# HopperLogger/HopperRender

Measured on AMD Instinct MI355X. Metric: interpolated frames/sec + ms/flow-calc, 2160p HDR, 1/2/4/8 MI355X, higher is better.
Workload: dtype u16

## Files before the change

### hopperrender_amd/csrc/hf_flow.hip

```cpp
#include <utility>
#include "hf_kernels.h"
#include "hf_phase_plane.h"

namespace hf {

thread_local LaunchObserver* t_launch_observer = nullptr;

namespace {

__device__ __forceinline__ int clampi(int v, int lo, int hi) { return min(max(v, lo), hi); }

__device__ __forceinline__ int rel_offset(int layer, int R) {
    const int d = layer - (R >> 1);
    return d > 0 ? d * d : -(d * d);
}

__device__ __forceinline__ int mirror_clamp(int p, int dim) {
    if (p >= dim) p = 2 * dim - p - 1; else if (p < 0) p = -p - 1;
    return clampi(p, 0, dim - 1);
}

template <typename E>
__global__ __launch_bounds__(256) void prep_phase_kernel(const PrepBatch batch, int H, int W, int S, PhaseLayout pl) {
    const E* __restrict__ f = (const E*)batch.frame[blockIdx.y];
// ... 802 lines not shown
        if (a.prev2.tx) {
            gx = table_at(a.prev2.tx, a.prev2, wx << a.cur.log2w, wy << a.cur.log2w);
            gy = table_at(a.prev2.ty, a.prev2, wx << a.cur.log2w, wy << a.cur.log2w);
        }
#pragma unroll
        for (int ax = 0; ax < 2; ax++)
#pragma unroll
            for (int v = 0; v < NV; v++) pre[ax][v] = tab0[ax * tab_axis + v];
        zx = wc.ox == gx; zy = wc.oy == gy;
    }
    if (a.pend.active) {
        const int tx0 = tile.tx * M::TW, ty0 = tile.ty * M::TH;
        const bool leader = tid == 0 && (tx0 & (a.pend.lvl.window - 1)) == 0 && (ty0 & (a.pend.lvl.window - 1)) == 0;
        const int v = resolve_pending(g, a, tx0, ty0, lane, leader);
        if (a.pend.axis) wc.oy = v; else wc.ox = v;
    }
    const int cap_cz = 7;
    uint32_t captured = 0;
    int off[2] = {wc.ox, wc.oy};

#pragma unroll
    for (int axis = 0; axis < 2; axis++) {
        bool reuse = zy && (axis == 0 ? zx : off[0] == wc.ox);
        if constexpr (G == 64) reuse = __builtin_amdgcn_readfirstlane((int)reuse) != 0;
        if (a.counters) {
            const bool lead = WS == 32 ? tid == 0 : G == 2 ? (lane & M::XM) == 0 : (lane & (G - 1)) == 0;
            const uint64_t mw = __builtin_amdgcn_ballot_w64(lead), mr = __builtin_amdgcn_ballot_w64(lead && reuse);
            if (lane == 0 && mw) {
                uint32_t* const c = a.counters + kCounterLevels + 4 * (a.level_index & 15) + 2 * axis;
                atomicAdd(c, (uint32_t)__builtin_popcountll(mw));
                if (mr) atomicAdd(c + 1, (uint32_t)__builtin_popcountll(mr));
            }
        }
        flow_v4* const tab = tab0 + axis * tab_axis;
        uint32_t tot[NOWN];
        int first = 0;
        if constexpr (PX == 4 && NR == 1) {
            uint32_t W[8];
            if (!reuse) {
                Strip<PX> strip[NR];
#pragma unroll
                for (int r = 0; r < NR; r++) strip[r] = load_strip<PX, true>(g, a, cx0, cy + r);
                uint32_t p[16];
#pragma unroll
                for (int cz = 0; cz < 16; cz++) p[cz] = 0u;
                bool from_lds = false;
                if constexpr (WS == 16 && SPLIT) {
                    if (axis == 1) from_lds = ysads_tile_try<16, 4, 1, true, kTabGroups>(p, g, a, strip[0].ref, off[0], off[1], cx0, cy, lane, s_rows);
                } else if constexpr (WS == 8 && SPLIT) {
                    if (axis == 1) from_lds = ysads_win8_try<true, kTabGroups>(p, g, a, strip[0].ref, off[0], off[1], cx0, cy, lane, s_rows);
                } else if constexpr (WS == 32) {
                    if (axis == 1) from_lds = ysads_tile_try<32, 8, 4, true, kTabGroups>(p, g, a, strip[0].ref, off[0], off[1], cx0 - lx, cy - ly, tid, s_rows);
                }
                if (!from_lds) strip_sads<4, G == 64, true, true, true, kTabGroups>(p, g, a, strip[0], off[0], off[1], axis);
                const uint32_t selw = (cy & 1) ? 0x07060302u : 0x05040100u;
#pragma unroll
                for (int j = 0; j < 8; j++) {
                    const uint32_t q0 = p[2 * j] + lane_xor<M::RM>(p[2 * j], lane);
                    const uint32_t q1 = p[2 * j + 1] + lane_xor<M::RM>(p[2 * j + 1], lane);
                    W[j] = __builtin_amdgcn_perm(q1, q0, selw);
                }
                if (a.sad_write) { tab[0] = flow_v4{W[0], W[1], W[2], W[3]}; tab[1] = flow_v4{W[4], W[5], W[6], W[7]}; }
            } else {
                const flow_v4 lo = pre[axis][0], hi = pre[axis][1];
                W[0] = lo.x; W[1] = lo.y; W[2] = lo.z; W[3] = lo.w; W[4] = hi.x; W[5] = hi.y; W[6] = hi.z; W[7] = hi.w;
            }
            first = packed_reduce<G, M::XM>(W, tot, lane);
        } else if constexpr (PX == 4) {
            uint32_t V[8];
            if (!reuse) {
                Strip<PX> strip[NR];
#pragma unroll
                for (int r = 0; r < NR; r++) strip[r] = load_strip<PX, true>(g, a, cx0, cy + r);
                uint32_t p[16];
#pragma unroll
                for (int cz = 0; cz < 16; cz++) p[cz] = 0u;
#pragma unroll
                for (int r = 0; r < NR; r++) strip_sads<4, false, true, true, true, kTabGroups>(p, g, a, strip[r], off[0], off[1], axis);
                uint32_t W0[8], W1[8];
#pragma unroll
                for (int j = 0; j < 8; j++) {
                    W0[j] = __builtin_amdgcn_perm(p[2 * j + 1], p[2 * j], 0x05040100u);
                    W1[j] = __builtin_amdgcn_perm(p[2 * j + 1], p[2 * j], 0x07060302u);
                    V[j] = W0[j] + W1[j];
                }
                if (a.sad_write) {
                    tab[0] = flow_v4{W0[0], W0[1], W0[2], W0[3]}; tab[1] = flow_v4{W0[4], W0[5], W0[6], W0[7]};
                    tab[2] = flow_v4{W1[0], W1[1], W1[2], W1[3]}; tab[3] = flow_v4{W1[4], W1[5], W1[6], W1[7]};
                }
            } else {
                const flow_v4 a0 = pre[axis][0], a1 = pre[axis][1], b0 = pre[axis][2 % NV], b1 = pre[axis][3 % NV];
                V[0] = a0.x + b0.x; V[1] = a0.y + b0.y; V[2] = a0.z + b0.z; V[3] = a0.w + b0.w;
                V[4] = a1.x + b1.x; V[5] = a1.y + b1.y; V[6] = a1.z + b1.z; V[7] = a1.w + b1.w;
            }
            first = packed_reduce<G, M::XM>(V, tot, lane);
        } else if constexpr (NR == 2) {
            if (!reuse) {
                Strip<PX> strip[NR];
#pragma unroll
                for (int r = 0; r < NR; r++) strip[r] = load_strip<PX, true>(g, a, cx0, cy + r);
#pragma unroll
                for (int cz = 0; cz < 16; cz++) tot[cz] = 0u;
#pragma unroll
                for (int r = 0; r < NR; r++) strip_sads<PX, false, true, false, true, kTabGroups>(tot, g, a, strip[r], off[0], off[1], axis);
            } else {
                unpack_u16x8(pre[axis][0], tot); unpack_u16x8(pre[axis][1 % NV], tot + 8);
            }
        } else {
            if (!reuse) {
                Strip<PX> strip[NR];
#pragma unroll
                for (int r = 0; r < NR; r++) strip[r] = load_strip<PX, true>(g, a, cx0, cy + r);
                uint32_t sad[16];
#pragma unroll
                for (int cz = 0; cz < 16; cz++) sad[cz] = 0u;
                strip_sads<PX, false, true, false, true, kTabGroups>(sad, g, a, strip[0], off[0], off[1], axis);
                butterfly_level<16, M::XM>(sad, lane);
#pragma unroll
                for (int k = 0; k < 8; k++) tot[k] = sad[k];
            } else {
                unpack_u16x8(pre[axis][0], tot);
            }
            first = (lane & M::XM) ? 8 : 0;
        }
        if constexpr (WS == 32) {
            if ((lane & 3) == 0) s_part[axis][wave][first] = tot[0];
            __syncthreads();
            tot[0] = s_part[axis][0][first] + s_part[axis][1][first] + s_part[axis][2][first] + s_part[axis][3][first];
        }
        const int best = group_argmin<G, true, M::XM>(tot, first, a, off[axis], axis ? wc.nby : wc.nbx, wc.npix, cap_cz,
                                                      axis == 0 && a.capture_delta, captured, lane);
        off[axis] = (int)(int16_t)(off[axis] + rel_offset(best, 16));
    }

    const bool leader = WS == 32 ? tid == 0 : G == 2 ? (lane & M::XM) == 0 : (lane & (G - 1)) == 0;
    HF_DBG_CHECK(wx >= 0 && wy >= 0 && wx < a.cur.nwx && wy < a.cur.nwy, 105);
    if (leader) {
        a.cur.tx[wy * a.cur.nwx + wx] = (int16_t)off[0];
        a.cur.ty[wy * a.cur.nwx + wx] = (int16_t)off[1];
        if (WS == 32 && a.still_count && off[0] == wc.ox && off[1] == wc.oy) atomicAdd(a.still_count, 1u);
        if (a.capture_delta && wx == 0 && wy == 0) *a.total_delta = captured / a.delta_divisor;
    }
}

template <bool FULL, bool R16, int NH>
__device__ __forceinline__ void flow_level32_wave_body(const Geom& g, const FlowStep& a, const TileId& tile, [[maybe_unused]] uint32_t* s_rows) {
    using M = Map<32>;
    const int R = R16 ? 16 : a.R;
    const int lane = (int)threadIdx.x;
    int lx, ly;
    M::at(lane, lx, ly);
    const int tx0 = tile.tx * M::TW, ty0 = tile.ty * M::TH;
    const int cx0 = tx0 + lx;
    const int wx = tx0 >> a.cur.log2w, wy = ty0 >> a.cur.log2w;
    WinConst wc = load_win_const(g, a, wx, wy, false);
    if (a.pend.active) {
        const bool leader = lane == 0 && (tx0 & (a.pend.lvl.window - 1)) == 0 && (ty0 & (a.pend.lvl.window - 1)) == 0;
        const int v = resolve_pending(g, a, tx0, ty0, lane, leader);
        if (a.pend.axis) wc.oy = v; else wc.ox = v;
    }
    const int cap_cz = (R >> 1) - 1;
    uint32_t captured = 0;
    int off[2] = {wc.ox, wc.oy};
#pragma unroll
    for (int axis = 0; axis < 2; axis++) {
        uint32_t sad[16];
#pragma unroll
        for (int cz = 0; cz < 16; cz++) sad[cz] = 0u;
        bool staged = false;
        if constexpr (FULL) if (axis == 1) {
            staged = ytile_can_stage<32>(g, a, __builtin_amdgcn_readfirstlane(off[1]), ty0);
            if (staged) with_rs(g.rs, [&](auto RS) { ystage_copy<decltype(RS)::value, 32, 8, 1>(a, __builtin_amdgcn_readfirstlane(off[0]), __builtin_amdgcn_readfirstlane(off[1]), tx0, ty0, lane, s_rows); });
        }
#pragma unroll 1
        for (int v = 0; v < 4; v++) {
            const Strip<4> strip = load_strip<4, FULL>(g, a, cx0, ty0 + ly + 8 * v);
            if (staged) with_rs(g.rs, [&](auto RS) { ystage_sads<decltype(RS)::value, 32, 8, 1, false, NH>(sad, a, strip.ref, __builtin_amdgcn_readfirstlane(off[0]), v * 64 + lane, s_rows); });
            else strip_sads<4, true, FULL, false, R16, NH>(sad, g, a, strip, off[0], off[1], axis);
        }
        const int first = group_reduce<64, 1>(sad, lane);
        const int best = group_argmin<64, R16, 1>(sad, first, a, off[axis], axis ? wc.nby : wc.nbx, wc.npix, cap_cz,
                                                  axis == 0 && a.capture_delta, captured, lane);
        off[axis] = (int)(int16_t)(off[axis] + rel_offset(best, R));
    }
    HF_DBG_CHECK(wx >= 0 && wy >= 0 && wx < a.cur.nwx && wy < a.cur.nwy, 105);
    if (lane == 0) {
        a.cur.tx[wy * a.cur.nwx + wx] = (int16_t)off[0];
        a.cur.ty[wy * a.cur.nwx + wx] = (int16_t)off[1];
        if (a.capture_delta && wx == 0 && wy == 0) *a.total_delta = captured / a.delta_divisor;
        if (a.still_count && off[0] == wc.ox && off[1] == wc.oy) atomicAdd(a.still_count, 1u);
    }
}

__device__ __forceinline__ void flow_level32_wave_tab_body(const Geom& g, const FlowStep& a, const TileId& tile, [[maybe_unused]] uint32_t* s_rows) {
    using M = Map<32>;
    const int lane = (int)threadIdx.x;
    int lx, ly;
    M::at(lane, lx, ly);
    const int tx0 = tile.tx * M::TW, ty0 = tile.ty * M::TH;
    const int cx0 = tx0 + lx, cy_0 = ty0 + ly;
    const int wx = tx0 >> a.cur.log2w, wy = ty0 >> a.cur.log2w;
    WinConst wc = load_win_const(g, a, wx, wy, false);
    const int nblk = a.sad_nbx * a.sad_nby;
    const int blk = (cy_0 >> 1) * a.sad_nbx + (cx0 >> 1) + (cy_0 & 1);
    HF_DBG_CHECK(blk >= 0 && blk + 12 * a.sad_nbx < nblk, 110);
    flow_v4* const tab0 = (flow_v4*)a.sadtab + (size_t)blk * 2;
    const size_t tab_axis = (size_t)nblk * 2, tab_round = (size_t)a.sad_nbx * 8;
    if (a.pend.active) {
        const bool leader = lane == 0 && (tx0 & (a.pend.lvl.window - 1)) == 0 && (ty0 & (a.pend.lvl.window - 1)) == 0;
        const int v = resolve_pending(g, a, tx0, ty0, lane, leader);
        if (a.pend.axis) wc.oy = v; else wc.ox = v;
    }
    const int cap_cz = 7;
    uint32_t captured = 0;
    int off[2] = {wc.ox, wc.oy};
    const uint32_t selw = (cy_0 & 1) ? 0x07060302u : 0x05040100u;
#pragma unroll
    for (int axis = 0; axis < 2; axis++) {
        if (a.counters && lane == 0) atomicAdd(a.counters + kCounterLevels + 4 * (a.level_index & 15) + 2 * axis, 1u);
        flow_v4* const tab = tab0 + axis * tab_axis;
        bool staged = false;
        if (axis == 1) {
            staged = ytile_can_stage<32>(g, a, __builtin_amdgcn_readfirstlane(off[1]), ty0);
            if (staged) with_rs(g.rs, [&](auto RS) { ystage_copy<decltype(RS)::value, 32, 8, 1>(a, __builtin_amdgcn_readfirstlane(off[0]), __builtin_amdgcn_readfirstlane(off[1]), tx0, ty0, lane, s_rows); });
        }
        uint32_t total = 0;
        int first = 0;
#pragma unroll 1
        for (int v = 0; v < 4; v++) {
            const Strip<4> strip = load_strip<4, true>(g, a, cx0, cy_0 + 8 * v);
            uint32_t p[16];
#pragma unroll
            for (int cz = 0; cz < 16; cz++) p[cz] = 0u;
            if (staged) with_rs(g.rs, [&](auto RS) { ystage_sads<decltype(RS)::value, 32, 8, 1, true, kTabGroups>(p, a, strip.ref, __builtin_amdgcn_readfirstlane(off[0]), v * 64 + lane, s_rows); });
            else strip_sads<4, true, true, true, true, kTabGroups>(p, g, a, strip, off[0], off[1], axis);
            uint32_t W[8];
#pragma unroll
            for (int j = 0; j < 8; j++) {
                const uint32_t q0 = p[2 * j] + lane_xor<M::RM>(p[2 * j], lane);
                const uint32_t q1 = p[2 * j + 1] + lane_xor<M::RM>(p[2 * j + 1], lane);
                W[j] = __builtin_amdgcn_perm(q1, q0, selw);
            }
            if (a.sad_write) { tab[v * tab_round] = flow_v4{W[0], W[1], W[2], W[3]}; tab[v * tab_round + 1] = flow_v4{W[4], W[5], W[6], W[7]}; }
            uint32_t t1[1];
            first = packed_reduce<64, 1>(W, t1, lane);
            total += t1[0];
        }
        const uint32_t tot[1] = {total};
        const int best = group_argmin<64, true, 1>(tot, first, a, off[axis], axis ? wc.nby : wc.nbx, wc.npix, cap_cz,
                                                   axis == 0 && a.capture_delta, captured, lane);
        off[axis] = (int)(int16_t)(off[axis] + rel_offset(best, 16));
    }
    HF_DBG_CHECK(wx >= 0 && wy >= 0 && wx < a.cur.nwx && wy < a.cur.nwy, 105);
    if (lane == 0) {
        a.cur.tx[wy * a.cur.nwx + wx] = (int16_t)off[0];
        a.cur.ty[wy * a.cur.nwx + wx] = (int16_t)off[1];
        if (a.still_count && off[0] == wc.ox && off[1] == wc.oy) atomicAdd(a.still_count, 1u);
        if (a.capture_delta && wx == 0 && wy == 0) *a.total_delta = captured / a.delta_divisor;
    }
}

template <bool TABK>
__global__ __launch_bounds__(64) void flow_level32_wave_kernel(const Geom g, const FlowBatchArgs batch) {
    const TileId tile = decode_tile<1>(batch, (g.lw + 31) / 32, (g.lh + 31) / 32);
    if (!tile.valid) return;
    const FlowStep a = member_step(batch, tile.pair);
    extern __shared__ __attribute__((aligned(16))) uint32_t s_rows[];
    const bool full = a.R == 16 && (tile.tx + 1) * 32 <= g.lw && (tile.ty + 1) * 32 <= g.lh;
    if constexpr (TABK) {
        if (full) flow_level32_wave_tab_body(g, a, tile, s_rows);
        else flow_level32_wave_body<false, true, kTabGroups>(g, a, tile, s_rows);
    }
    else if (full) flow_level32_wave_body<true, true, 1>(g, a, tile, s_rows);
    else if (a.R == 16) flow_level32_wave_body<false, true, 1>(g, a, tile, s_rows);
    else flow_level32_wave_body<false, false, 1>(g, a, tile, s_rows);
}

template <int WS, bool SPLIT, bool ROWS1 = false, bool TABK = false>
__global__ __launch_bounds__(SPLIT ? 64 : 256) void flow_level_small_kernel(const Geom g, const FlowBatchArgs batch) {
    using M = typename MapSel<WS, ROWS1>::type;
    const TileId tile = decode_tile<SPLIT ? M::WAVES : 1>(batch, (g.lw + M::TW - 1) / M::TW, (g.lh + M::TH - 1) / M::TH);
    if (!tile.valid) return;
    const FlowStep a = member_step(batch, tile.pair);
    static_assert(!SPLIT || WS <= 16, "a 32x32 window is shared by the four waves of a workgroup");
    __shared__ uint32_t s_part[SPLIT ? 1 : 2][4][16];
    extern __shared__ __attribute__((aligned(16))) uint32_t s_rows[];
    const bool full = a.R == 16 && (tile.tx + 1) * M::TW <= g.lw && (tile.ty + 1) * M::TH <= g.lh;
    if constexpr (TABK) {
        const bool tab = full && (M::TW == 32 || ((tile.tx * M::TW) | 31) < g.lw);
        if (tab) {
            const int tid = SPLIT ? (int)(tile.wave * 64 + threadIdx.x) : (int)threadIdx.x;
            int lx, ly;
            M::at(tid, lx, ly);
            flow_level_tab_body<WS, SPLIT, ROWS1>(g, a, tile.tx * M::TW + lx, tile.ty * M::TH + ly, lx, ly, tid, tile, s_part, s_rows);
        }
        else if (full) flow_level_small_body<WS, SPLIT, true, ROWS1, true, kTabGroups>(g, a, tile, s_part, s_rows);
        else flow_level_small_body<WS, SPLIT, false, ROWS1, true, kTabGroups>(g, a, tile, s_part, s_rows);
    }
    else if (full) flow_level_small_body<WS, SPLIT, true, ROWS1>(g, a, tile, s_part, s_rows);
    else if (a.R == 16) flow_level_small_body<WS, SPLIT, false, ROWS1, true>(g, a, tile, s_part, s_rows);
    else flow_level_small_body<WS, SPLIT, false, ROWS1>(g, a, tile, s_part, s_rows);
}

template <int WPB, bool FULL, bool R16 = FULL>
__device__ __forceinline__ void flow_big_partial_body(const Geom& g, const FlowStep& a, const TileId& tile, uint32_t (*s_part)[16], [[maybe_unused]] uint32_t* s_rows) {
    const int R = R16 ? 16 : a.R;
    const int tid = threadIdx.x, wave = tid >> 6, lane = tid & 63;
    const int lx = (tid & 15) * 4, ly = tid >> 4;
    const int tx0 = tile.tx * 64, ty0 = tile.ty * (4 * WPB);
    const int cx0 = tx0 + lx, cy = ty0 + ly;
    const int wx = tx0 >> a.cur.log2w, wy = ty0 >> a.cur.log2w;
    int ox = 0, oy = 0;
    if (a.prev.tx) {
        ox = table_at(a.prev.tx, a.prev, wx << a.cur.log2w, wy << a.cur.log2w);
        oy = table_at(a.prev.ty, a.prev, wx << a.cur.log2w, wy << a.cur.log2w);
    }
    if (a.pend.active) {
        const bool leader = tid == 0 && (tx0 & (a.pend.lvl.window - 1)) == 0 && (ty0 & (a.pend.lvl.window - 1)) == 0;
        const int v = resolve_pending(g, a, tx0, ty0, lane, leader);
        if (a.pend.axis) oy = v; else ox = v;
    } else if (a.axis == 1) {
        ox = a.cur.tx[wy * a.cur.nwx + wx];
    }
    const Strip<4> strip = load_strip<4, FULL>(g, a, cx0, cy);
    uint32_t sad[16];
#pragma unroll
    for (int cz = 0; cz < 16; cz++) sad[cz] = 0u;
    bool from_lds = false;
    if constexpr (FULL && WPB == 4) if (a.axis == 1) from_lds = ysads_tile_try<16, 16, 4>(sad, g, a, strip.ref, ox, oy, tx0, ty0, tid, s_rows);
    if (!from_lds) strip_sads<4, true, FULL, false, R16>(sad, g, a, strip, ox, oy, a.axis);
    const int first = group_reduce<64>(sad, lane);
    HF_DBG_CHECK(wx >= 0 && wy >= 0 && wx < a.cur.nwx && wy < a.cur.nwy, 106);
    uint32_t* dst = &a.sums[(wy * a.cur.nwx + wx) * 16];
    if constexpr (WPB == 1) {
        if ((lane & 3) == 0 && first < R) atomicAdd(dst + first, sad[0]);
    } else {
        if ((lane & 3) == 0) s_part[wave][first] = sad[0];
        __syncthreads();
        if (tid < R) {
            uint32_t t = 0;
#pragma unroll
            for (int w = 0; w < WPB; w++) t += s_part[w][tid];
            atomicAdd(dst + tid, t);
        }
    }
}

template <int WPB>
__global__ __launch_bounds__(64 * WPB) void flow_big_partial_kernel(const Geom g, const FlowBatchArgs batch) {
    constexpr int TW = 64, TH = 4 * WPB;
    const TileId tile = decode_tile<1>(batch, (g.lw + TW - 1) / TW, (g.lh + TH - 1) / TH);
    if (!tile.valid) return;
    const FlowStep a = member_step(batch, tile.pair);
    __shared__ uint32_t s_part[WPB][16];
    extern __shared__ __attribute__((aligned(16))) uint32_t s_rows[];
    const bool full = a.R == 16 && (tile.tx + 1) * TW <= g.lw && (tile.ty + 1) * TH <= g.lh;
    if (full) flow_big_partial_body<WPB, true>(g, a, tile, s_part, s_rows);
    else if (a.R == 16) flow_big_partial_body<WPB, false, true>(g, a, tile, s_part, s_rows);
    else flow_big_partial_body<WPB, false>(g, a, tile, s_part, s_rows);
}

__global__ __launch_bounds__(256) void flow_big_argmin_kernel(const Geom g, const FlowBatchArgs batch) {
    const FlowStep a = member_step(batch, (int)blockIdx.y);
    const int lane16 = threadIdx.x & 15;
    const int nwin = a.cur.nwx * a.cur.nwy;
    for (int w = blockIdx.x * 16 + (threadIdx.x >> 4); w < nwin; w += gridDim.x * 16) {
        const int wy = w / a.cur.nwx, wx = w - wy * a.cur.nwx;
        const WinConst wc = load_win_const(g, a, wx, wy, a.axis == 1);
        const int searched0 = a.axis ? wc.oy : wc.ox;
        Best b{0xFFFFFFFFu, 16};
        uint32_t mine = 0;
        if (lane16 < a.R) {
            const int cand = (int)(int16_t)(searched0 + rel_offset(lane16, a.R));
            mine = (a.sums[w * 16 + lane16] << a.delta_scalar) +
                   wc.npix * window_bias(cand, a.use_neighbors, a.axis ? wc.nby : wc.nbx, a.neighbor_scalar);
            b.sum = mine; b.cz = lane16;
        }
        const int lane = (int)(threadIdx.x & 63);
        best_xor<1>(b, lane); best_xor<2>(b, lane); best_xor<4>(b, lane); best_xor<8>(b, lane);
        if (lane16 == 0) {
            int16_t* t = a.axis ? a.cur.ty : a.cur.tx;
            t[w] = (int16_t)(searched0 + rel_offset(b.cz, a.R));
        }
        if (a.capture_delta && w == 0 && lane16 == (a.R >> 1) - 1) *a.total_delta = mine / a.delta_divisor;
    }
}

__global__ void expand_offsets_kernel(const Geom g, const FlowLevel L, int16_t* __restrict__ out) {
    const int x = blockIdx.x * 64 + (threadIdx.x & 63), y = blockIdx.y * 4 + (threadIdx.x >> 6);
    if (x >= g.lw || y >= g.lh) return;
    const size_t p = (size_t)y * g.lw + x, N = (size_t)g.lw * g.lh;
    out[p] = L.tx ? (int16_t)table_at(L.tx, L, x, y) : (int16_t)0;
    out[N + p] = L.ty ? (int16_t)table_at(L.ty, L, x, y) : (int16_t)0;
}

}

PhaseLayout make_phase_layout(const Geom& g, int max_iterations) {
    PhaseLayout pl{};
    pl.rs = g.rs;
    pl.nph = 1 << g.rs;
    pl.nph2 = pl.nph > 1 ? pl.nph / 2 : 1;
    const int reach = (max_iterations + 1) * 64 + 8;
    pl.mx = (((reach >> g.rs) + 2 + 3) / 4) * 4;
    pl.lwp = ((g.lw + 2 * pl.mx + 4 + 31) / 32) * 32;
    pl.bytes = (size_t)g.H * pl.nph2 * pl.lwp * sizeof(uint32_t);
    return pl;
}

template <typename E>
static bool launch_prep_fast(const Geom& g, const PhaseLayout& pl, const PrepBatch& b, hipStream_t stream) {
    const int lw = g.W >> g.rs;
    const size_t row_bytes = (size_t)g.in_stride * sizeof(E);
    if ((lw << g.rs) != g.W || lw != g.lw || (lw & 3) || pl.mx > lw || (pl.mx & 3) || (row_bytes & 15) || (pl.lwp & 3) || g.rs > 4 || (g.H & 1))
        return false;
    for (int i = 0; i < b.n; i++) if (((uintptr_t)b.frame[i]) & 15) return false;
    const dim3 grd((lw / 4 + 127) / 128, g.H / 2, b.n);
    const bool nt = b.n > 1;
    switch (g.rs) {
        case 0: if (nt) HF_LAUNCH("plane", (prep_phase_fast_kernel<E, 0, true>), grd, dim3(128), 0, stream, b, g.H, g.W, g.in_stride, pl); else HF_LAUNCH("plane", (prep_phase_fast_kernel<E, 0, false>), grd, dim3(128), 0, stream, b, g.H, g.W, g.in_stride, pl); break;
        case 1: if (nt) HF_LAUNCH("plane", (prep_phase_fast_kernel<E, 1, true>), grd, dim3(128), 0, stream, b, g.H, g.W, g.in_stride, pl); else HF_LAUNCH("plane", (prep_phase_fast_kernel<E, 1, false>), grd, dim3(128), 0, stream, b, g.H, g.W, g.in_stride, pl); break;
        case 2: if (nt) HF_LAUNCH("plane", (prep_phase_fast_kernel<E, 2, true>), grd, dim3(128), 0, stream, b, g.H, g.W, g.in_stride, pl); else HF_LAUNCH("plane", (prep_phase_fast_kernel<E, 2, false>), grd, dim3(128), 0, stream, b, g.H, g.W, g.in_stride, pl); break;
        case 3: if (nt) HF_LAUNCH("plane", (prep_phase_fast_kernel<E, 3, true>), grd, dim3(128), 0, stream, b, g.H, g.W, g.in_stride, pl); else HF_LAUNCH("plane", (prep_phase_fast_kernel<E, 3, false>), grd, dim3(128), 0, stream, b, g.H, g.W, g.in_stride, pl); break;
        default: if (nt) HF_LAUNCH("plane", (prep_phase_fast_kernel<E, 4, true>), grd, dim3(128), 0, stream, b, g.H, g.W, g.in_stride, pl); else HF_LAUNCH("plane", (prep_phase_fast_kernel<E, 4, false>), grd, dim3(128), 0, stream, b, g.H, g.W, g.in_stride, pl); break;
    }
    return true;
}

void launch_prep_frames(const Geom& g, const PhaseLayout& pl, const PrepBatch& b, hipStream_t stream) {
    if (g.hdr ? launch_prep_fast<uint16_t>(g, pl, b, stream) : launch_prep_fast<uint8_t>(g, pl, b, stream)) return;
    const size_t smem = 2 * (size_t)((g.W + 15) / 16) * 16;
    const dim3 grd(g.H, b.n);
    if (g.hdr) HF_LAUNCH("plane", (prep_phase_kernel<uint16_t>), grd, dim3(256), smem, stream, b, g.H, g.W, g.in_stride, pl);
    else HF_LAUNCH("plane", (prep_phase_kernel<uint8_t>), grd, dim3(256), smem, stream, b, g.H, g.W, g.in_stride, pl);
}

template <typename E>
__global__ __launch_bounds__(256) void prep_grid_kernel(const PrepBatch batch, int H, int S, PhaseLayout pl, int lw) {
    const E* __restrict__ f = (const E*)batch.frame[blockIdx.z];
    uint32_t* __restrict__ pp = batch.pp[blockIdx.z];
    const int j = blockIdx.x * 256 + threadIdx.x;
    if (j >= lw) return;
    const int sy = (int)blockIdx.y << pl.rs, x = j << pl.rs;
    HF_DBG_CHECK(sy < H && x + 1 < S && ((size_t)sy * pl.nph2 * pl.lwp + pl.mx + j + 1) * 4 <= pl.bytes, 107);
    const E* __restrict__ yr = f + (size_t)sy * S + x;
    const E* __restrict__ cr = f + (size_t)H * S + (size_t)(sy >> 1) * S + x;
    typedef E e2 __attribute__((ext_vector_type(2)));
    const e2 y2 = __builtin_nontemporal_load((const e2*)yr), c2 = __builtin_nontemporal_load((const e2*)cr);
    pp[(size_t)sy * pl.nph2 * pl.lwp + pl.mx + j] = pack_element(top8<E>(y2.x), top8<E>(y2.y), top8<E>(c2.x), top8<E>(c2.y));
}

void launch_prep_grid(const Geom& g, const PhaseLayout& pl, const PrepBatch& b, hipStream_t stream) {
    const dim3 grd((g.lw + 255) / 256, g.lh, b.n);
    if (g.hdr) HF_LAUNCH("grid_samples", (prep_grid_kernel<uint16_t>), grd, dim3(256), 0, stream, b, g.H, g.in_stride, pl, g.lw);
    else HF_LAUNCH("grid_samples", (prep_grid_kernel<uint8_t>), grd, dim3(256), 0, stream, b, g.H, g.in_stride, pl, g.lw);
}

void launch_prep_frame(const Geom& g, const PhaseLayout& pl, const void* frame, uint32_t* pp, hipStream_t stream) {
    PrepBatch b{};
    b.n = 1; b.frame[0] = frame; b.pp[0] = pp;
    launch_prep_frames(g, pl, b, stream);
}

constexpr int kRowPerLaneMaxBatch = 4;
#ifndef HF_LEVEL32_ONE_WAVE_MIN_BATCH
#define HF_LEVEL32_ONE_WAVE_MIN_BATCH 4
#endif
constexpr int kLevel32OneWaveMinBatch = HF_LEVEL32_ONE_WAVE_MIN_BATCH;
void launch_flow_level_small(const Geom& g, const FlowBatch& b, hipStream_t stream) {
    const int ws = b.s[0].cur.window;
    const bool rows1 = b.n <= kRowPerLaneMaxBatch && ws <= 4;
    const int tw = rows1 && ws == 2 ? MapRow<2>::TW : 32;
    const int tiles_x = (g.lw + tw - 1) / tw, tiles_y = (g.lh + 31) / 32;
    FlowBatchArgs kb = pack_batch(b, tiles_x, tiles_y);
    const size_t lds = b.s[0].R != 16 ? 0 : ws == 32 ? ystage_bytes<32, 8, 4>(g.rs) : ws == 16 ? ystage_bytes<16, 4, 1>(g.rs) : ws == 8 ? win8_stage_bytes(g.rs) : 0;
    const dim3 grd(xcd_grid(tiles_x, tiles_y, 1, b.n));
    auto split = [&](int waves) { return dim3(xcd_grid(tiles_x, tiles_y, waves, b.n)); };
    kb.common.y_rows_lds = lds != 0;
    const bool tabk = b.s[0].sadtab && b.s[0].R == 16 && (b.s[0].sad_read || b.s[0].sad_write);
#define HF_LEVEL(NAME, WS_, SPLIT_, ROWS1_, GRID, BLOCK, LDS)                                                                            \
    do {                                                                                                                                 \
        if (tabk) HF_LAUNCH(NAME, (flow_level_small_kernel<WS_, SPLIT_, ROWS1_, true>), GRID, BLOCK, LDS, stream, g, kb);                \
        else HF_LAUNCH(NAME, (flow_level_small_kernel<WS_, SPLIT_, ROWS1_, false>), GRID, BLOCK, LDS, stream, g, kb);                    \
    } while (0)
    switch (ws) {
        case 32:
            if (b.n >= kLevel32OneWaveMinBatch) {
                const size_t lds1 = b.s[0].R != 16 ? 0 : ystage_bytes<32, 8, 1>(g.rs);
                kb.common.y_rows_lds = lds1 != 0;
                if (tabk) HF_LAUNCH("level_32", (flow_level32_wave_kernel<true>), grd, dim3(64), lds1, stream, g, kb);
                else HF_LAUNCH("level_32", (flow_level32_wave_kernel<false>), grd, dim3(64), lds1, stream, g, kb);
                break;
            }
            HF_LEVEL("level_32", 32, false, false, grd, dim3(256), lds);
            break;
        case 16: HF_LEVEL("level_16", 16, true, false, split(Map<16>::WAVES), dim3(64), lds); break;
        case 8: HF_LEVEL("level_8", 8, true, false, split(Map<8>::WAVES), dim3(64), lds); break;
        case 4:
            if (rows1) HF_LEVEL("level_4", 4, true, true, split(MapRow<4>::WAVES), dim3(64), 0);
            else HF_LEVEL("level_4", 4, true, false, split(Map<4>::WAVES), dim3(64), 0);
            break;
        default:
            if (rows1) HF_LEVEL("level_2", 2, true, true, split(MapRow<2>::WAVES), dim3(64), 0);
            else HF_LEVEL("level_2", 2, true, false, split(Map<2>::WAVES), dim3(64), 0);
            break;
    }
#undef HF_LEVEL
}

#ifndef HF_BIG_ONE_WAVE_MIN_BATCH
#define HF_BIG_ONE_WAVE_MIN_BATCH 4
#endif
constexpr int kBigWavesPerBlock = 4, kBigOneWaveMinBatch = HF_BIG_ONE_WAVE_MIN_BATCH, kBigOneWaveMinRs = 2;
void launch_flow_big_partial(const Geom& g, const FlowBatch& b, hipStream_t stream) {
    const bool y = b.s[0].axis == 1;
    const char* name = y ? "large_windows_y" : "large_windows_x";
    const int wpb = b.n >= kBigOneWaveMinBatch && g.rs >= kBigOneWaveMinRs ? 1 : kBigWavesPerBlock;
    const int tiles_x = (g.lw + 63) / 64, tiles_y = (g.lh + 4 * wpb - 1) / (4 * wpb);
    const dim3 grd(xcd_grid(tiles_x, tiles_y, 1, b.n));
    const size_t lds = y && b.s[0].R == 16 && wpb == 4 ? ystage_bytes<16, 16, 4>(g.rs) : 0;
    FlowBatchArgs kb = pack_batch(b, tiles_x, tiles_y);
    kb.common.y_rows_lds = lds != 0;
    if (wpb == 1) HF_LAUNCH(name, (flow_big_partial_kernel<1>), grd, dim3(64), lds, stream, g, kb);
    else HF_LAUNCH(name, (flow_big_partial_kernel<kBigWavesPerBlock>), grd, dim3(64 * kBigWavesPerBlock), lds, stream, g, kb);
}

void launch_flow_big_argmin(const Geom& g, const FlowBatch& b, hipStream_t stream) {
    const int nwin = b.s[0].cur.nwx * b.s[0].cur.nwy;
    HF_LAUNCH("large_windows_argmin", flow_big_argmin_kernel, dim3((nwin + 15) / 16, b.n), dim3(256), 0, stream, g, pack_batch(b, 1, 1));
}

bool dbg_bounds_read_flow(unsigned out[5], bool reset) {
#ifdef HF_DEBUG_BOUNDS
    unsigned rec[5] = {0, 0, 0, 0, 0};
    if (hipMemcpyFromSymbol(rec, HIP_SYMBOL(g_dbg_bounds), sizeof(rec)) != hipSuccess) return false;
    if (rec[0] && !out[0]) for (int i = 1; i < 5; i++) out[i] = rec[i];
    out[0] += rec[0];
    if (reset) { const unsigned zero[5] = {0, 0, 0, 0, 0}; (void)hipMemcpyToSymbol(HIP_SYMBOL(g_dbg_bounds), zero, sizeof(zero)); }
    return true;
#else
    (void)out; (void)reset;
    return false;
#endif
}

void launch_expand_offsets(const Geom& g, const FlowLevel& last, int16_t* out, hipStream_t stream) {
    const dim3 grd((g.lw + 63) / 64, (g.lh + 3) / 4);
    expand_offsets_kernel<<<grd, 256, 0, stream>>>(g, last, out);
}

}
```

Baseline: 89430.

## Process runs of row tiles per one-wave block in large-window flow kernel

In the one-wave-per-block path of the large-window partial SAD kernel, each block now walks a run of several 4-row strips inside the same window, accumulating SADs in registers with the next strip prefetched, so fewer blocks launch and fewer atomics hit the window sums. For the y axis with full tiles, it also stages the shifted comparison rows in LDS per 16-row chunk and computes the SADs from LDS. The catch is fewer blocks in flight, which can hurt occupancy, plus extra LDS use and barriers in the one-wave path.

Measured after the change: 90040, median of 6. Within noise of the previous version (+0.7%).

```diff
diff --git a/hopperrender_amd/csrc/hf_flow.hip b/hopperrender_amd/csrc/hf_flow.hip
--- a/hopperrender_amd/csrc/hf_flow.hip
+++ b/hopperrender_amd/csrc/hf_flow.hip
@@ -1128,12 +1128,24 @@
     else flow_level_small_body<WS, SPLIT, false, ROWS1>(g, a, tile, s_part, s_rows);
 }
 
+#ifndef HF_BIG_RUN_TILES
+#define HF_BIG_RUN_TILES 4
+#endif
+#ifndef HF_BIG_RUN_YROWS_LDS
+#define HF_BIG_RUN_YROWS_LDS 1
+#endif
+constexpr int kBigRunTiles = HF_BIG_RUN_TILES;
+constexpr bool kBigRunYRowsLds = HF_BIG_RUN_YROWS_LDS != 0;
+static_assert(kBigRunTiles == 1 || kBigRunTiles == 2 || kBigRunTiles == 4 || kBigRunTiles == 8 || kBigRunTiles == 16, "a run of tiles never crosses a 64-row window");
+__host__ __device__ constexpr int big_run_tiles(int wpb) { return wpb == 1 ? kBigRunTiles : 1; }
+
 template <int WPB, bool FULL, bool R16 = FULL>
 __device__ __forceinline__ void flow_big_partial_body(const Geom& g, const FlowStep& a, const TileId& tile, uint32_t (*s_part)[16], [[maybe_unused]] uint32_t* s_rows) {
     const int R = R16 ? 16 : a.R;
     const int tid = threadIdx.x, wave = tid >> 6, lane = tid & 63;
     const int lx = (tid & 15) * 4, ly = tid >> 4;
-    const int tx0 = tile.tx * 64, ty0 = tile.ty * (4 * WPB);
+    constexpr int RUN = big_run_tiles(WPB);
+    const int tx0 = tile.tx * 64, ty0 = tile.ty * (4 * WPB * RUN);
     const int cx0 = tx0 + lx, cy = ty0 + ly;
     const int wx = tx0 >> a.cur.log2w, wy = ty0 >> a.cur.log2w;
     int ox = 0, oy = 0;
@@ -1148,13 +1160,47 @@
     } else if (a.axis == 1) {
         ox = a.cur.tx[wy * a.cur.nwx + wx];
     }
-    const Strip<4> strip = load_strip<4, FULL>(g, a, cx0, cy);
     uint32_t sad[16];
 #pragma unroll
     for (int cz = 0; cz < 16; cz++) sad[cz] = 0u;
-    bool from_lds = false;
-    if constexpr (FULL && WPB == 4) if (a.axis == 1) from_lds = ysads_tile_try<16, 16, 4>(sad, g, a, strip.ref, ox, oy, tx0, ty0, tid, s_rows);
-    if (!from_lds) strip_sads<4, true, FULL, false, R16>(sad, g, a, strip, ox, oy, a.axis);
+    if constexpr (WPB == 1) {
+        const int nt = FULL ? RUN : min(RUN, (g.lh - ty0 + 3) >> 2);
+        const bool cols_inside = tx0 + 64 <= g.lw;
+        auto inside = [&](int t) { return FULL || (R16 && cols_inside && ty0 + 4 * t + 4 <= g.lh); };
+        auto load = [&](int t) { return inside(t) ? load_strip<4, true>(g, a, cx0, cy + 4 * t) : load_strip<4, false>(g, a, cx0, cy + 4 * t); };
+        bool from_lds = false;
+        if constexpr (FULL && kBigRunYRowsLds && RUN % 4 == 0) {
+            if (a.axis == 1 && ytile_can_stage<4 * RUN>(g, a, __builtin_amdgcn_readfirstlane(oy), ty0)) {
+                from_lds = true;
+                const int oxu = __builtin_amdgcn_readfirstlane(ox), oyu = __builtin_amdgcn_readfirstlane(oy);
+                with_rs(g.rs, [&](auto RS) {
+                    constexpr int rs = decltype(RS)::value;
+                    for (int c = 0; c < RUN / 4; c++) {
+                        Strip<4> s4[4];
+#pragma unroll
+                        for (int t = 0; t < 4; t++) s4[t] = load_strip<4, true>(g, a, cx0, cy + 16 * c + 4 * t);
+                        if (c) __syncthreads();
+                        ystage_copy<rs, 16, 16, 1>(a, oxu, oyu, tx0, ty0 + 16 * c, lane, s_rows);
+#pragma unroll
+                        for (int t = 0; t < 4; t++) ystage_sads<rs, 16, 16, 1>(sad, a, s4[t].ref, oxu, t * 64 + lane, s_rows);
+                    }
+                });
+            }
+        }
+        Strip<4> strip = load(0);
+        for (int t = 0; t < (from_lds ? 0 : nt); t++) {
+            Strip<4> next = strip;
+            if (t + 1 < nt) next = load(t + 1);
+            if (inside(t)) strip_sads<4, true, true, false, true>(sad, g, a, strip, ox, oy, a.axis);
+            else if constexpr (!FULL) strip_sads<4, true, false, false, R16>(sad, g, a, strip, ox, oy, a.axis);
+            strip = next;
+        }
+    } else {
+        const Strip<4> strip = load_strip<4, FULL>(g, a, cx0, cy);
+        bool from_lds = false;
+        if constexpr (FULL) if (a.axis == 1) from_lds = ysads_tile_try<16, 16, 4>(sad, g, a, strip.ref, ox, oy, tx0, ty0, tid, s_rows);
+        if (!from_lds) strip_sads<4, true, FULL, false, R16>(sad, g, a, strip, ox, oy, a.axis);
+    }
     const int first = group_reduce<64>(sad, lane);
     HF_DBG_CHECK(wx >= 0 && wy >= 0 && wx < a.cur.nwx && wy < a.cur.nwy, 106);
     uint32_t* dst = &a.sums[(wy * a.cur.nwx + wx) * 16];
@@ -1174,7 +1220,7 @@
 
 template <int WPB>
 __global__ __launch_bounds__(64 * WPB) void flow_big_partial_kernel(const Geom g, const FlowBatchArgs batch) {
-    constexpr int TW = 64, TH = 4 * WPB;
+    constexpr int TW = 64, TH = 4 * WPB * big_run_tiles(WPB);
     const TileId tile = decode_tile<1>(batch, (g.lw + TW - 1) / TW, (g.lh + TH - 1) / TH);
     if (!tile.valid) return;
     const FlowStep a = member_step(batch, tile.pair);
@@ -1342,9 +1388,10 @@
     const bool y = b.s[0].axis == 1;
     const char* name = y ? "large_windows_y" : "large_windows_x";
     const int wpb = b.n >= kBigOneWaveMinBatch && g.rs >= kBigOneWaveMinRs ? 1 : kBigWavesPerBlock;
-    const int tiles_x = (g.lw + 63) / 64, tiles_y = (g.lh + 4 * wpb - 1) / (4 * wpb);
+    const int th = 4 * wpb * big_run_tiles(wpb);
+    const int tiles_x = (g.lw + 63) / 64, tiles_y = (g.lh + th - 1) / th;
     const dim3 grd(xcd_grid(tiles_x, tiles_y, 1, b.n));
-    const size_t lds = y && b.s[0].R == 16 && wpb == 4 ? ystage_bytes<16, 16, 4>(g.rs) : 0;
+    const size_t lds = !(y && b.s[0].R == 16) ? 0 : wpb == 4 ? ystage_bytes<16, 16, 4>(g.rs) : kBigRunYRowsLds ? ystage_bytes<16, 16, 1>(g.rs) : 0;
     FlowBatchArgs kb = pack_batch(b, tiles_x, tiles_y);
     kb.common.y_rows_lds = lds != 0;
     if (wpb == 1) HF_LAUNCH(name, (flow_big_partial_kernel<1>), grd, dim3(64), lds, stream, g, kb);
```
